# luntergroup/smcsmc

Hardware: AMD Instinct MI355X
Metric: genome segments/sec per EM iteration (Np=10000, 2 diploids, 100 Mb) (higher is better)
Workload: dtype f64

## Files before the change

include/smcsmc_pf.h:

```cpp
#ifndef SMCSMC_PF_H
#define SMCSMC_PF_H
#include <stdint.h>

#ifdef __cplusplus
extern "C" {
#endif

typedef struct pf_model {
    int32_t n_epochs;
    int32_t n_pops;
    int32_t nsam;
    int32_t flags;
    double loci_length;
    double mutation_rate;
    double recombination_rate;
    const double* change_times;
    const double* pop_sizes;
    const double* mig_rates;
    const double* single_mig;
    const int32_t* sample_pops;
    const int32_t* record_flags;
    const double* lags;
    int32_t n_bias_heights;
    int32_t delay_type;
// ... 8 lines not shown
    const double* rate_values;
    const double* leaf_rel_rates;
} pf_model;

typedef struct pf_params {
    int64_t np;
    double ess_fraction;
    uint64_t seed;
    int32_t max_trace_events;
    int32_t flags;
    int64_t log_cap;
    int64_t gen_cap;
    int64_t piece_cap;
    int32_t debug;
    int32_t mig_cap;
    int32_t count_wgs;
    int32_t delay_cap;
    int32_t count_workers;
    int32_t reserved4;
} pf_params;
#define PF_DEBUG_FORCE_LDS 1
#define PF_DEBUG_NO_FUSE   2
#define PF_DEBUG_NO_COUNT  4
#define PF_DEBUG_TWO_LAUNCH 8
#define PF_DEBUG_NO_SPEC_STAGE 32
#define PF_DEBUG_K_PIPE   16

#define PF_DEBUG_NO_DRAW_TABLE 128

#define PF_DEBUG_NO_SEARCH_LUT 256

#define PF_DEBUG_ONE_LAUNCH (1 << 23)

#define PF_DEBUG_NO_PAIR 4096
#define PF_DEBUG_FORCE_WIDE 2048

typedef struct pf_segments {
    int64_t n;
    const double* start;
    const double* length;
    const int8_t* state;
    const int8_t* alleles;
    const int32_t* max_record_epoch;
} pf_segments;

typedef struct pf_lookahead {
    int32_t level;
    int32_t max_doubletons;
    int32_t n_quantiles;
    int32_t flags;
    int64_t n;
    const double* first_singleton_distance;
    const double* relative_mutation_rate;
    const int8_t* is_singleton_unphased;
    const int32_t* n_doubletons;
    const int8_t* doubleton_idx;
    const double* doubleton_dist;
    const double* first_split_distance;
    const int8_t* split_alleles;
    const int32_t* split_count;
    const double* quantiles;
    const double* tbl_lengths;
    double mean_total_branch_length;
} pf_lookahead;
#define PF_LA_ROW_PIPELINE 1
#define PF_LA_ROW_PIPELINE_MP 2
// ... 92 lines not shown
```

profiles/gaps.py:

```python
#!/usr/bin/env python3
import csv
import glob
import statistics
import sys
from collections import defaultdict

path = glob.glob(sys.argv[1] + "/**/*kernel_trace.csv", recursive=True)[0]
rows = list(csv.DictReader(open(path)))
byq = defaultdict(list)
for r in rows:
    byq[r["Queue_Id"]].append((int(r["Start_Timestamp"]), int(r["End_Timestamp"]), r["Kernel_Name"].split("(")[0][:40]))
for q, ks in sorted(byq.items(), key=lambda kv: -len(kv[1]))[:3]:
    ks.sort()
    gaps = defaultdict(list)
    for (s0, e0, n0), (s1, e1, n1) in zip(ks, ks[1:]):
        gaps[(n0, n1)].append(s1 - e0)
    busy = sum(e - s for s, e, _ in ks)
    span = ks[-1][1] - ks[0][0]
    print("queue %s: %d kernels, busy %.1f ms of %.1f ms" % (q, len(ks), busy / 1e6, span / 1e6))
    for (a, b), g in sorted(gaps.items(), key=lambda kv: -len(kv[1]))[:6]:
        print("   %-40s -> %-40s n=%6d  gap mean %8.2f us  median %8.2f us" % (a, b, len(g), statistics.mean(g) / 1e3, statistics.median(g) / 1e3))
```

smcsmc_amd/csrc/pf_hip.hip:

```cpp
#include <hip/hip_runtime.h>
#include <type_traits>
#include <hip/hip_ext.h>

#include <algorithm>
#include <atomic>
#include <cmath>
#include <cstdio>
#include <cstdlib>
#include <cstring>
#include <mutex>
#include <string>
#include <vector>

#include "../../include/smcsmc_pf.h"
#include "pf_device.h"
#include "pf_types.h"
#include "pf_lane.h"
#include "pf_tree_reg.h"
#include "pf_look_reg.h"
#include "pf_lds_body.h"
#include "pf_mp_host.h"
#include "pf_wide_host.h"
#include "pf_pipe.h"
#include "pf_lds_pipe.h"
// ... 1370 lines not shown
#define PF_CNT_WIDE 128
#define PF_CNT_BATCH 2

template <int NI, int P, class KA>
__device__ __forceinline__ void count_run(AccT<P>& acc, const KA& A, const CountSrc& Q, const Win& W, const LMap& L, int g, long long i,
                                          int nr, const int* rst, const int* ran, double inv) {
    const long long Np = A.Np;
    int q0 = rst[i];
    int q1 = i + 1 < nr ? rst[i + 1] : (int)Np;
    long long a = ran[i];
    if (q1 <= q0 || q1 > (int)Np || q0 < 0 || a < 0 || a >= Np) return;
    const double* offp = Q.offp;
    const double* scp_ = Q.scanp;
    double hi = offp[(q1 - 1) >> 6] + scp_[q1 - 1];
    double lo = q0 > 0 ? offp[(q0 - 1) >> 6] + scp_[q0 - 1] : 0.0;
    double w = (hi - lo) * inv;
    if (!(w > 0.0)) return;
    unsigned k0 = A.gstart[(size_t)(g % A.Gcap) * Np + a];
    unsigned k1 = A.gstart[(size_t)((g + 1) % A.Gcap) * Np + a];
    if (Q.widx_live[a] - k0 > A.cap || k1 - k0 > A.cap) { if (!A.ctrl->err) A.ctrl->err = ERR_LOG_OVERFLOW; return; }
    records_contrib<NI, P>(acc, A, W, L, w, a, k0, k1);
}

struct FlatTask { double w; int a; unsigned k0; };
__device__ __forceinline__ FlatTask* count_flat_tasks() {
    __shared__ FlatTask ft[PF_BS];
    return ft;
}
__device__ __forceinline__ int* count_flat_prefix() {
    __shared__ int pre[PF_BS + 1];
    return pre;
}

template <int NM, int P, bool EXACT = false, class KA>
__device__ __forceinline__ void count_body(const KA& A, const CountSrc& Q, int e, double win_a, double win_b, int bx, int nbxg) {
    constexpr int NI = NM - 1;
    using AC = AccT<P>;
    constexpr int LDS_BYTES = (int)(((sizeof(AC) * (PF_BS / 64) + 15) & ~(size_t)15) + sizeof(int) * (PF_CNT_TILE + 1 + PF_BS / 64) + 16);
    char* const cl = count_lds<LDS_BYTES>();
    AC* const red = (AC*)cl;
    int* const s_off = (int*)(cl + ((sizeof(AC) * (PF_BS / 64) + 15) & ~(size_t)15));
    int* const s_wsum = s_off + PF_CNT_TILE + 1;
    const long long Np = A.Np;
    const int n = EXACT ? NM : A.n;
    const int G = Q.G;
    const double inv = Q.inv;
    Win W;
    W.e = e; W.rf = A.recflags[e];
    W.T0 = A.T[e]; W.T1 = e + 1 < A.E ? A.T[e + 1] : PF_INF;
    W.a_e = win_a; W.b_e = win_b;
    W.end_seq = (A.L == W.b_e);
    double* const s_lbins = count_bins();
    LMap L;
    L.lds = s_lbins; L.b0 = (long long)(W.a_e / 100.0); L.gopp = A.lmap_opp; L.gcnt = A.lmap_cnt; L.nbins = A.lmap_bins;
    {
        const long long span = (long long)(W.b_e / 100.0) - L.b0 + 4;
        L.nlds = span < 1 ? 1 : (span > PF_LBINS ? PF_LBINS : (int)span);
        L.ncnt = (A.n + 3) * L.nlds <= PF_LBINS ? L.nlds : 0;
    }
    bool bins_ready = false;
    const int g_lo = Q.g_lo, g_hi = Q.g_hi;
    if (g_hi < g_lo) return;
    const int lane = threadIdx.x & 63;
    const long long gtid = (long long)bx * PF_BS + threadIdx.x;
    const long long nthreads = (long long)nbxg * PF_BS;
    AC acc;
#pragma unroll
    for (int k = 0; k < AC::NC; ++k) acc.v[k] = 0.0;
    for (int tile_hi = g_hi; tile_hi >= g_lo; tile_hi -= PF_CNT_TILE) {
        const int tile_lo = tile_hi - PF_CNT_TILE + 1 > g_lo ? tile_hi - PF_CNT_TILE + 1 : g_lo;
// ... 116 lines not shown
                const double* rec = rec_ptr(A, a_r, s_ft[lo_j].k0 + (unsigned)(r - s_fpre[lo_j]));
                double f0 = rec[0], f1 = rec[1], f2 = rec[2], f3 = rec[3], f4 = rec[4];
                double S[NI];
#pragma unroll
                for (int q = 0; q < NI; ++q) S[q] = q < n - 1 ? rec[5 + q] : 0.0;
                unsigned long long dw = 0;
                if constexpr (NI >= PF_NMAX) if (L.gopp) dw = (unsigned long long)__double_as_longlong(rec[4 + n]);
                record_contrib_one<NI, P>(acc, A, W, L, w_r, a_r, f0, f1, f2, f3, f4, S, dw);
            }
            __syncthreads();
        }
    }
    if (L.gopp && bins_ready) {
        __syncthreads();
        for (int k = threadIdx.x; k < L.nlds; k += PF_BS) {
            double v = s_lbins[k];
            long long idx = L.b0 + k;
            if (v != 0.0 && idx < L.nbins) atomicAdd(&L.gopp[idx], v);
        }
        for (int k = threadIdx.x; k < (A.n + 2) * L.ncnt; k += PF_BS) {
            const double v = s_lbins[L.nlds + k];
            const long long idx = L.b0 + k % L.ncnt;
            if (v != 0.0 && idx < L.nbins) atomicAdd(&L.gcnt[(size_t)(k / L.ncnt) * L.nbins + idx], v);
        }
    }
#pragma unroll
    for (int k = 0; k < AC::NC; ++k) acc.v[k] = wave_tree_sum(acc.v[k]);
    if ((threadIdx.x & 63) == 0) red[threadIdx.x >> 6] = acc;
    __syncthreads();
    if (threadIdx.x < AC::NC) {
        const int k = threadIdx.x;
        double t = red[0].v[k];
        for (int w = 1; w < PF_BS / 64; ++w) t += red[w].v[k];
        A.partial[((size_t)e * A.nbx + bx) * AC::NC + k] += t;
    }
}


template <int NM, int P>
__global__ __launch_bounds__(PF_BS) void k_count(KArgs A, int e0, Windows Wn) {
    const int e = e0 + (int)blockIdx.y;
    if (e < Wn.first || e >= A.E) return;
    count_body<NM, P>(A, count_src_parity(A, A.sp, e), e, Wn.a[e], Wn.b[e], (int)blockIdx.x, (int)gridDim.x);
}

template <int NM, int P>
__global__ __launch_bounds__(PF_BS) void k_count_cw(KArgs A, int e0, Windows Wn) {
    const int e = e0 + (int)blockIdx.y;
    if (e < Wn.first || e >= A.E) return;
    const int j = A.E - 1 - e;
    const int cnb = A.cw_off[j + 1] - A.cw_off[j];
    if ((int)blockIdx.x >= cnb) return;
    count_body<NM, P>(A, count_src_parity(A, A.sp, e), e, Wn.a[e], Wn.b[e], (int)blockIdx.x, cnb);
}

template <int NM, bool BIASED, bool EXACT, bool TREES = false>
__global__ __launch_bounds__(PF_BS) void k_row(KArgs A, long long s, int fuse, int nb, int count_first, Windows Wprev) {
    if ((int)blockIdx.x < nb) {
        extend_reg_body<NM, BIASED, EXACT, TREES>(A, s, fuse);
    } else {
        const int idx = (int)blockIdx.x - nb;
        const int e = count_first + idx / nb;
        if (e < Wprev.first || e >= A.E) return;
        count_body<NM, 1, EXACT>(A, count_src_parity(A, A.sp ^ 1, e), e, Wprev.a[e], Wprev.b[e], idx % nb, nb);
    }
}

// ... 248 lines not shown
        c->gen_prev = c->gen; c->nres_prev = c->n_resample;
        if (PL.b_set_cur >= 0) c->cur = PL.b_set_cur;
    }
}

template <class KA>
__device__ __forceinline__ void draw_role(const KA& A, int tb, int nT, int par) {
    const long long Np = A.Np;
    const unsigned long long* c_in = A.dt_ctr + (size_t)(par ^ 1) * Np;
    const unsigned long long* f_in = A.dt_filled + (size_t)(par ^ 1) * Np;
    unsigned long long* f_out = A.dt_filled + (size_t)par * Np;
    const unsigned long long seed = A.seed;
    for (long long p = (long long)tb * PF_BS + threadIdx.x; p < Np; p += (long long)nT * PF_BS) {
        const unsigned long long c0 = c_in[p], f_old = f_in[p];
        const unsigned long long to = c0 + PF_DRAW_RING;
        double2* tab = (double2*)A.dt_tab + (size_t)p * PF_DRAW_RING;
        for (unsigned long long cc = f_old > c0 ? f_old : c0; cc < to; ++cc) {
            double u0, u1;
            philox_pair(seed, (unsigned)p, 0u, cc, u0, u1);
            tab[(unsigned)cc & (PF_DRAW_RING - 1)] = make_double2(u0, -dlog(u1));
        }
        f_out[p] = to;
    }
}

template <class KA>
__device__ __forceinline__ void pipe_ledger_item(const KA& A, const PipeLaunch& PL, const Ctrl::RowInfo& r, int lb) {
    const RunLists src = run_lists(A, r.lver), dst = run_lists(A, r.lver ^ 1);
    const int nblk = PL.nblk;
    if (lb < nblk) ledger_new_list(A, dst, A.rg_blkcnt + (size_t)PL.lc_slot * nblk * A.blk_gran, nblk, lb, r.gen, A.blk_gran);
    else ledger_update(A, lb - nblk, PL.nL - nblk, r.gen, r.g_retain, src, dst);
}

template <int NM, bool EXACT, int P, class KA>
__device__ __forceinline__ void pipe_count_item(const KA& A, const PipeLaunch& PL, const Ctrl::RowInfo& r, int idx) {
    int e, cbx, cnb;
    if (A.cw_off && !(A.flags & 512)) {
        int j = 0, hi = A.E;
        while (hi - j > 1) { const int mid = (j + hi) >> 1; if (A.cw_off[mid] <= idx) j = mid; else hi = mid; }
        e = A.E - 1 - j; cbx = idx - A.cw_off[j]; cnb = A.cw_off[j + 1] - A.cw_off[j];
    } else {
        e = (A.flags & 512) ? r.first + idx / PL.ncw : A.E - 1 - idx / PL.ncw;
        cbx = idx % PL.ncw; cnb = PL.ncw;
    }
    if (e >= A.E || e < r.first) return;
    if (A.flags & (1 << 22)) return;
    const DState st = state_slot(A, PL.lc_slot);
    CountSrc Q;
    Q.w = st.w_post; Q.S = st.S; Q.xm = st.x_mark; Q.ml = st.mark_limit;
    Q.widx = A.rg_widx + (size_t)PL.lc_slot * A.Np;
    Q.widx_live = A.rg_widx + (size_t)PL.live_slot * A.Np;
    Q.scanp = A.rg_scanp + (size_t)PL.lc_slot * A.Np;
    Q.offp = A.rg_coffp + (size_t)PL.lc_slot * A.nc;
    Q.lists = run_lists(A, r.lver);
    Q.inv = r.inv_T; Q.G = r.gen; Q.g_lo = r.g_lo[e]; Q.g_hi = r.g_hi[e];
    count_body<NM, P, EXACT>(A, Q, e, r.wa[e], r.wb[e], cbx, cnb);
}

template <int NM, bool BIASED, bool EXACT, bool TREES, int P = 1, bool BLC = false, bool QUEUE = false, bool LEAN = false, bool NO_EXTEND = false, bool LOOK = false, class KA>
__device__ __forceinline__ void pipe_roles(const KA& A, long long s, const PipeLaunch& PL, const Windows& Wb) {
    const int bx = pf_bx();
    const int nb = PL.nb;
    if constexpr (!LEAN) {
        if (bx < nb) {
            if constexpr (P == 1 && !BLC && !NO_EXTEND) { if (PL.row.extend || PL.row.complete) extend_reg_body<NM, BIASED, EXACT, TREES, true, false, LOOK>(A, s, 0, PL.row); }
            return;
        }
        if (bx == nb) {
            if (PL.b_slot < 0) return;
            extern __shared__ double smem[];
            PipeLds q = pipe_carve(smem + (2 * PF_EPAD + A.E + 2 * PF_BIAS_MAX + 3), A.nc);
            pipe_bookkeeping<BIASED>(A, q, PL, Wb);
            return;
        }
        if (bx - (nb + 1) < PL.nT) {
            if constexpr (P == 1 && !BLC) draw_role(A, bx - (nb + 1), PL.nT, PL.row.draws - 1);
            return;
        }
    } else {
        if (bx <= nb) return;
    }
    if (PL.lc_slot < 0 || PL.nL < -1) return;
    const Ctrl* c = A.ctrl;
    const Ctrl::RowInfo& r = c->ri[PL.lc_slot];
    const int lb = bx - (nb + 1) - PL.nT;
    if constexpr (!QUEUE) {
        if (lb < PL.nL) { if (r.flag) pipe_ledger_item(A, PL, r, lb); }
        else pipe_count_item<NM, EXACT, P>(A, PL, r, lb - PL.nL);
    } else {
        __shared__ int s_wk[8];
        if (lb >= PL.workers) return;
        if (threadIdx.x == 0) { s_wk[0] = PL.lc_slot; s_wk[1] = PL.live_slot; s_wk[2] = PL.nL; s_wk[3] = PL.nblk; s_wk[4] = PL.ncw; }
        const KA* Ap = &A;
        for (;;) {
            asm volatile("" : "+s"(Ap));
            const KA& A2 = *Ap;
            __syncthreads();
            if (threadIdx.x == 0) s_wk[6] = (int)__hip_atomic_fetch_add(&A2.ctrl->wq[s_wk[0]], 1u, __ATOMIC_RELAXED, __HIP_MEMORY_SCOPE_AGENT);
            __syncthreads();
            PipeLaunch Q2;
            Q2.lc_slot = s_wk[0]; Q2.live_slot = s_wk[1]; Q2.nL = s_wk[2]; Q2.nblk = s_wk[3]; Q2.ncw = s_wk[4];
            const int it = s_wk[6];
            const Ctrl::RowInfo& r2 = A2.ctrl->ri[Q2.lc_slot];
            const int ncnt = r2.first < A2.E ? (A2.cw_off ? A2.cw_off[A2.E - r2.first] : (A2.E - r2.first) * Q2.ncw) : 0;
            if (it >= ncnt + (r2.flag ? Q2.nL : 0)) return;
            if (it < ncnt) pipe_count_item<NM, EXACT, P>(A2, Q2, r2, it);
            else pipe_ledger_item(A2, Q2, r2, it - ncnt);
        }
    }
}

template <int NM, bool BIASED, bool EXACT, bool TREES>
__global__ __launch_bounds__(PF_BS) void k_pipe(KArgs A, long long s, PipeLaunch PL, Windows Wb) {
    pipe_roles<NM, BIASED, EXACT, TREES>(A, s, PL, Wb);
}

template <class KA>
__device__ __forceinline__ void sweep_windows(const KA& A, Ctrl* c, double pos, Windows& W) {
    const int e = threadIdx.x, E = A.E;
    if (e < 64) {
        const bool in = e < E;
// ... 57 lines not shown
        PipeLaunch PL;
        if (sweep_plan(ch, s, nb, PL)) {
            if (ch.split == 2) PL.nL = -3;
            if (pf_bx() == nb && PL.b_slot >= 0) sweep_windows(A, A.ctrl, PL.b_pos, W);
            pipe_roles<NM, BIASED, EXACT, TREES, 1, false, QUEUE, false, HEAD, LOOK>(A, s, PL, W);
        }
    }
    if constexpr (TRACE) {
        __syncthreads();
        if (threadIdx.x == 0) if (unsigned long long* w = wg_trace_slot(ch, t)) w[1] = wall_clock64();
    }
}
template <int NM, bool BIASED, bool EXACT, bool TREES, bool LOOK = false>
__global__ __launch_bounds__(PF_BS) void k_sweep(const SweepChunk* tab_g, long long t, int nb) {
    sweep_kernel_body<NM, BIASED, EXACT, TREES, false, false, false, LOOK>(tab_g, t, nb);
}
template <bool EXACT, bool TREES>
__global__ __launch_bounds__(PF_BS) __attribute__((amdgpu_waves_per_eu(3, 3))) void k_sweep4(const SweepChunk* tab_g, long long t, int nb) {
    sweep_kernel_body<4, false, EXACT, TREES, false, false, true>(tab_g, t, nb);
}
template <bool EXACT>
__global__ __launch_bounds__(PF_BS) void k_sweep4p(const SweepChunk* tab_g, long long t, int nb) {
    sweep_kernel_body<4, false, EXACT, false, false, false, true, false, true>(tab_g, t, nb);
}
template <bool EXACT, bool TRACE>
__global__ __launch_bounds__(PF_BS) __attribute__((amdgpu_waves_per_eu(3, 3))) void k_sweep4q(const SweepChunk* tab_g, long long t, int nb) {
    sweep_kernel_body<4, false, EXACT, false, TRACE, true, true>(tab_g, t, nb);
}
template <bool EXACT>
__global__ __launch_bounds__(PF_BS) __attribute__((amdgpu_waves_per_eu(3, 3))) void k_sweep4t(const SweepChunk* tab_g, long long t, int nb) {
    sweep_kernel_body<4, false, EXACT, false, true, false, true>(tab_g, t, nb);
}

template <int NM, int P, bool BIASED, bool EXACT = false, bool LEAN = false, bool QUEUE = false>
__device__ __forceinline__ void sweep_blc_body(const SweepChunk* tab_g, long long t) {
    SweepChunkC* tab = (SweepChunkC*)tab_g;
    SweepChunkC& ch = tab[pf_chunk()];
    KArgsC& A = ch.A;
    const long long s = ch.s_begin + t;
    __shared__ Windows W;
    Ctrl* c = A.ctrl;
    PipeLaunch PL;
    if (sweep_plan(ch, s, 0, PL)) {
        PL.nT = 0;
        if (ch.split == 2) PL.b_slot = -1;
        if (pf_bx() == 0 && PL.b_slot >= 0) sweep_windows(A, c, PL.b_pos, W);
        pipe_roles<NM, BIASED, EXACT, false, P, true, QUEUE, LEAN>(A, s, PL, W);
    }
}

template <int NM, int P, bool BIASED>
__global__ __launch_bounds__(PF_BS) void k_sweep_blc(const SweepChunk* tab_g, long long t) {
    sweep_blc_body<NM, P, BIASED>(tab_g, t);
}
template <bool EXACT>
__global__ __launch_bounds__(PF_BS) __attribute__((amdgpu_waves_per_eu(4, 4))) void k_sweep_blc4(const SweepChunk* tab_g, long long t) {
    sweep_blc_body<4, 1, false, EXACT, true>(tab_g, t);
}
template <bool EXACT>
__global__ __launch_bounds__(PF_BS) __attribute__((amdgpu_waves_per_eu(4, 4))) void k_sweep_blc4q(const SweepChunk* tab_g, long long t) {
    sweep_blc_body<4, 1, false, EXACT, true, true>(tab_g, t);
}

template <bool BIASED>
__global__ __launch_bounds__(PF_BS) void k_sweep_xl(const SweepChunk* tab_g, long long t) {
    SweepChunkC* tab = (SweepChunkC*)tab_g;
    SweepChunkC& ch = tab[pf_chunk()];
    KArgsC& A = ch.A;
    const long long s = ch.s_begin + t;
    PipeLaunch PL;
    if (!sweep_plan(ch, s, 0, PL)) return;
    if (!(PL.row.extend || PL.row.complete)) return;
    extern __shared__ double smem[];
    extend_lds_pipe_body<BIASED>(A, s, PL.row, smem);
}

__global__ void k_sweep_seed(const SweepChunk* tab_g) {
    SweepChunkC* tab = (SweepChunkC*)tab_g;
    SweepChunkC& ch = tab[blockIdx.x];
    KArgsC& A = ch.A;
    if (ch.s_last < ch.s_begin) return;
    Ctrl* c = A.ctrl;
    const int slot = (int)((ch.s_begin + PF_RING - 1) & (PF_RING - 1));
    if (threadIdx.x == 0) {
        Ctrl::RowInfo& r = c->ri[slot];
        r.n_res = c->n_resample; r.gen = c->gen; r.flag = 0; r.lver = c->lver; r.g_retain = c->g_retain; r.first = A.E;
        r.inv_T = 1.0; r.T = 1.0; r.S1 = 0.0; r.u = 0.0; r.pos = c->cur_pos;
        c->xr[slot].n_res = c->n_resample; c->xr[slot].gen = c->gen; c->xr[slot].flag = 0;
    }
    if ((int)threadIdx.x < A.E) c->counted_to[threadIdx.x] = ch.counted_to[threadIdx.x];
// ... 383 lines not shown
```

smcsmc_amd/csrc/pf_pipe.h:

```cpp
#pragma once
#include <cstddef>
#include <cstring>
#include <type_traits>

#include "pf_device.h"
#include "pf_types.h"

#define PF_PIPE_BS 256

__device__ __forceinline__ KArgsC& pf_reopen(KArgsC& A) { KArgsC* q = &A; asm volatile("" : "+s"(q)); return *q; }
__device__ __forceinline__ const KArgs& pf_reopen(const KArgs& A) { return A; }

#define PF_PIPE_STAGE 16
struct RowDecision { double T, S1, S2, ess, inv, u; int flag; };
struct PipeLds {
    double* l2s;
    double* pmx;
    double* l2_post; double* l2_sq; double* l2_tot;
    double* wredd;
    double* stage;
    int* slo;
    int* wint;
};
__host__ __device__ inline size_t pipe_lds_doubles(int nc) {
// ... 194 lines not shown
        else if constexpr (L == 1) return (unsigned)l1[K];
        else if constexpr (L == 2) return (unsigned)l2[K];
        else if constexpr (L == 3) return (unsigned)l3[K];
        else return (unsigned)l4[K];
    }
    template <int OFF> __device__ __forceinline__ unsigned long long dword() const {
        return ((unsigned long long)word<OFF + 4>() << 32) | (unsigned long long)word<OFF>();
    }
};
#define PF_HP(R, f) ((__attribute__((address_space(1))) std::remove_pointer_t<decltype(SweepHead::f)>*)(R).template dword<(int)offsetof(SweepHead, f)>())
#define PF_HL(R, f) ((long long)(R).template dword<(int)offsetof(SweepHead, f)>())
#define PF_HI(R, f) ((int)(R).template word<(int)offsetof(SweepHead, f)>())

inline SweepHead sweep_head_entry(const KArgs& A, const SweepChunk& ch, int phase) {
    SweepHead H;
    memset(&H, 0, sizeof(H));
    const size_t sp = (size_t)((ch.s_begin + phase + PF_RING - 1) & (PF_RING - 1)), Np = (size_t)A.Np, nc = (size_t)A.nc;
    H.s_begin = ch.s_begin; H.s_last = ch.s_last; H.Np = A.Np;
    H.nc = A.nc; H.n = A.n; H.E = A.E; H.flags = A.flags; H.nT = ch.nT; H.split = ch.split; H.nblk = ch.nblk; H.no_count = ch.no_count; H.P = A.P;
    H.slot_prev = (int)sp;
    H.cpost = A.rg_cpost + sp * nc; H.csq = A.rg_csq + sp * nc; H.cpil = A.rg_cpil + sp * nc; H.cmx1 = A.rg_cmx1 + sp * nc;
    H.last1 = &A.ctrl->last1[sp]; H.xr_before = &A.ctrl->xr[(sp + PF_RING - 1) & (PF_RING - 1)];
    H.scan1m = A.rg_scan1m + sp * Np; H.rg_widx = A.rg_widx + sp * Np;
    const DState st = state_slot(A, (int)sp);
    H.S = st.S; H.C = st.C; H.w_post = st.w_post; H.w_pilot = st.w_pilot; H.next_base = st.next_base; H.x_mark = st.x_mark;
    H.mark_limit = st.mark_limit; H.Ltree = st.Ltree;
    H.widx = A.widx; H.rng_ctr = A.rng_ctr; H.ebuf = A.ebuf;
    H.dt_filled = A.dt_filled ? A.dt_filled + (size_t)((ch.s_begin + phase + 1) & 1) * Np : nullptr;
    H.seg_start = A.seg_start; H.seg_len = A.seg_len; H.seg_limit = A.seg_limit; H.seg_state = A.seg_state; H.seg_alleles = A.seg_alleles;
    H.T = A.T; H.Hc = A.Hc; H.inv2N = A.inv2N; H.lut = A.lut; H.ctrl = A.ctrl;
    return H;
}

template <class KA>
__device__ __forceinline__ double sweep_seg_pos(const KA& A, long long s) {
    const double e = A.seg_start[s] + A.seg_len[s];
    return e < A.L ? e : A.L;
}

__device__ __forceinline__ bool sweep_plan(SweepChunkC& ch, long long s, int nb, PipeLaunch& PL) {
    const long long s_begin = ch.s_begin, s_last = ch.s_last;
    if (s_last < s_begin || s > s_last + 2) return false;
    const bool extend = s <= s_last, flush1 = s == s_last + 1;
    const bool have_b = extend ? (s > s_begin) : flush1;
    const bool have_lc = extend ? (s > s_begin + 1) : (flush1 ? (s_last - 1 >= s_begin) : true);
    PL.nb = nb; PL.nblk = ch.nblk;
    PL.row.extend = extend ? 1 : 0;
    PL.row.complete = ((extend && s > s_begin) || flush1) ? 1 : 0;
    PL.row.slot_prev = PL.row.complete ? (int)((s - 1) & (PF_RING - 1)) : -1;
    PL.row.slot_out = (int)(s & (PF_RING - 1));
    PL.row.pos_prev = (PL.row.complete && s > s_begin) ? sweep_seg_pos(ch.A, s - 1) : 0.0;
    PL.row.draws = ch.nT > 0 ? 1 + (int)(s & 1) : 0;
    PL.ahead = PL.row.ahead = (ch.split || ch.A.P > 1) ? 1 : 0;
    PL.nT = extend ? ch.nT : 0;
    PL.b_slot = have_b ? (int)((s - 1) & (PF_RING - 1)) : -1;
    PL.b_row = s - 1;
    PL.b_pos = have_b ? sweep_seg_pos(ch.A, s - 1) : 0.0;
    PL.b_set_cur = flush1 ? (int)((s_last + 1) & (PF_RING - 1)) : -1;
    PL.lc_slot = (have_lc && !ch.no_count) ? (int)((s - 2) & (PF_RING - 1)) : -1;
    PL.live_slot = (int)((s - 1) & (PF_RING - 1));
    PL.nL = PL.lc_slot >= 0 ? ch.nL_full : 0;
    PL.ncw = ch.ncw;
    PL.workers = ch.workers;
    return true;
}
```

smcsmc_amd/csrc/pf_run.h:

```cpp

static Windows host_windows(pf_handle* h, double current_base, bool end_data) {
    const int E = h->E;
    Windows W;
    memset(&W, 0, sizeof(W));
    W.first = E;
    W.end_data = end_data ? 1 : 0;
    for (int e = 0; e < E; ++e) {
        double lagging = end_data ? 0.0 : h->h_lags[e];
        double x_end = current_base - lagging;
        W.a[e] = h->h_counted_to[e];
        if ((x_end - h->h_counted_to[e]) < lagging * 0.1 && W.first > e) {
            W.b[e] = h->h_counted_to[e];
        } else {
            W.b[e] = x_end;
            W.first = std::min(W.first, e);
        }
    }
    for (int e = 0; e < E; ++e) h->h_counted_to[e] = W.b[e];
    return W;
}

static bool timing_on(pf_handle* h, long long s) { return h->timing_period > 0 && (s % h->timing_period) == 0; }

static Windows no_windows(pf_handle* h) {
// ... 391 lines not shown
            ch.s_last = last;
            for (int q = 0; q < h->E; ++q) ch.counted_to[q] = g->h_counted_to[q];
            ch.no_count = g->no_count ? 1 : 0;
            ch.nL_full = nL_full;
            ch.ncw = g->ncw;
            ch.nblk = g->nblocks;
            ch.nT = (g->A.dt_tab && g->P == 1) ? g->nblocks : 0;
            ch.split = split;
            ch.workers = g->workers;
            ch.trace = h->d_trace; ch.trace_t0 = h->trace_t0; ch.trace_n = h->d_trace ? h->trace_n : 0; ch.trace_stride = h->trace_stride;
            if (last >= s_begin) steps = std::max(steps, last - s_begin + 3);
        }
        if (steps == 0) return 0;
        const size_t head_bytes = sizeof(SweepHead) * PF_RING * (size_t)nh, chunk_bytes = sizeof(SweepChunk) * (size_t)nh;
        h->h_table.assign(head_bytes + chunk_bytes, 0);
        SweepHead* heads_end = (SweepHead*)(h->h_table.data() + head_bytes);
        if (h->P == 1 && h->n <= 4 && !is_biased(h))
            for (int k = 0; k < nh; ++k)
                for (int j = 0; j < PF_RING; ++j) *sweep_head_of(heads_end, k, j) = sweep_head_entry(h->h_sweep[k].A, h->h_sweep[k], j);
        memcpy(h->h_table.data() + head_bytes, h->h_sweep.data(), chunk_bytes);
        if (hipMemcpyAsync((char*)h->d_sweep - head_bytes, h->h_table.data(), head_bytes + chunk_bytes, hipMemcpyHostToDevice, h->stream) != hipSuccess) {
            g_err = "upload of the chunk table failed"; return -1;
        }
        hipLaunchKernelGGL(k_sweep_seed, dim3(nh), dim3(PF_BS), 0, h->stream, h->d_sweep);
        if (two_streams) {
            seeded = next_sync_event(h);
            hipEventRecord(seeded, h->stream);
        }
        W1.resize((size_t)nh); W2.resize((size_t)nh);
        for (int k = 0; k < nh; ++k) { W1[k] = no_windows(hs[k]); W2[k] = W1[k]; }
        return 1;
    }
    void ring_wait(long long t) const {
        static_assert(PF_RING == 16, "the wait schedule is written for sixteen ring slots");
        if (t >= 8 && (t & 7) == 0) hipStreamWaitEvent(h->stream, h->ev_blc[(size_t)((t - 7) & 15)], 0);
    }
    hipEvent_t x_done(long long t) const { return h->ev_x[(size_t)(t & 15)]; }
    hipEvent_t blc_done(long long t) const { return h->ev_blc[(size_t)(t & 15)]; }
    int lc_wgs(long long t) const {
        int columns = 0;
        bool any_lc = false;
        for (int k = 0; k < nh; ++k)
            if (t >= 2 && s_begin + t - 2 <= h->h_sweep[k].s_last && !hs[k]->no_count) { any_lc = true; columns = std::max(columns, h->E - W2[k].first); }
        const int workers = h->h_sweep[0].workers;
        return workers > 0 ? (any_lc ? workers : 0) : nL_full + h->cw_off[columns];
    }
    void step_done(long long t) {
        if ((t & 1023) == 1023) trim_spans(h);
        const long long s = s_begin + t;
        for (int k = 0; k < nh; ++k) {
            pf_handle* g = hs[k];
            W2[k] = W1[k];
            if (s <= h->h_sweep[k].s_last) {
                W1[k] = host_windows(g, seg_pos(g, s), false);
                g->step_windows = W1[k];
                if (W1[k].first < g->E && !g->no_count) g->fin_pending = true;
            } else {
                W1[k] = no_windows(g);
            }
        }
    }
    int leave() {
        h->k_launches[0] -= 2;
        if (two_streams) hipStreamWaitEvent(h->stream, blc_done(steps - 1), 0);
        for (int k = 0; k < nh; ++k) {
            pf_handle* g = hs[k];
            const long long last = h->h_sweep[k].s_last;
            if (last >= s_begin) g->seg_done = last + 1;
            if (k > 0) {
// ... 26 lines not shown
            Timed tm(h, 0, timing_on(h, s_begin + t));
            launch_sweep(h, grid, t);
        }
        if (check_launch("k_sweep")) return -1;
        F.step_done(t);
    }
    return F.leave();
}

static int run_sweep_split(pf_handle* const* hs, int nh, long long s_begin, long long s_end) {
    if (s_begin >= s_end) return 0;
    SweepFrame F(hs, nh, s_begin, true);
    pf_handle* h = F.h;
    const int nb = F.nb;
    if (F.join()) return -1;
    if (const int rc = F.table(s_end, 2); rc <= 0) return rc;
    const int nbp = (int)((h->Np + PF_PAIR_N - 1) / PF_PAIR_N);
    bool paired = !dbg(h, PF_DEBUG_NO_PAIR) && (long long)nh * nbp <= pf_device_cus(h->device);
    for (int k = 0; k < nh; ++k) if (hs[k]->A.vb_coal || dbg(hs[k], PF_DEBUG_NO_PAIR)) paired = false;
    for (int k = 0; k < nh; ++k) hs[k]->row_form = paired ? PF_ROW_FORM_PAIRED : PF_ROW_FORM_SINGLE;
    const int nbx = paired ? nbp : nb;
    if (paired && !h->pair_lds_set) {
        hipError_t rc = hipSuccess;
        with_row_instance(h, [&](auto NM, auto BIASED, auto EXACT, auto TREES) {
            if constexpr (NM == 4 && !BIASED && !TREES) rc = hipFuncSetAttribute((const void*)k_sweep4p<EXACT>, hipFuncAttributeMaxDynamicSharedMemorySize, (int)h->smem_pipe);
        });
        if (rc != hipSuccess) { g_err = "k_sweep4p: the LDS of the paired row kernel was refused (PF_DEBUG_NO_PAIR runs the other form)"; return -1; }
        h->pair_lds_set = true;
    }
    const dim3 gx((unsigned)(nbx + 1 + h->h_sweep[0].nT), (unsigned)nh), blk(PF_BS);
    const long long batch = std::max(1, std::min(4, h->split_batch > 0 ? h->split_batch : 4));
    std::vector<unsigned> pending_grid((size_t)batch, 1u);
    const bool queue = h->h_sweep[0].workers > 0;
    hipStreamWaitEvent(h->cstream, F.seeded, 0);
    for (long long t = 0; t < F.steps; ++t) {
        F.ring_wait(t);
        const bool batch_end = ((t + 1) % batch) == 0 || t == F.steps - 1;
        {
            Timed tm(h, 0, timing_on(h, s_begin + t));
            with_row_instance(h, [&](auto NM, auto BIASED, auto EXACT, auto TREES) {
                if constexpr (NM == 4 && !BIASED && !TREES) {
                    if (paired) {
                        if (batch_end) hipExtLaunchKernelGGL((k_sweep4p<EXACT>), gx, blk, h->smem_pipe, h->stream, nullptr, F.x_done(t), 0, h->d_sweep, t, nbx);
                        else hipLaunchKernelGGL((k_sweep4p<EXACT>), gx, blk, h->smem_pipe, h->stream, h->d_sweep, t, nbx);
                    } else if (batch_end) hipExtLaunchKernelGGL((k_sweep4<EXACT, false>), gx, blk, h->smem_pipe, h->stream, nullptr, F.x_done(t), 0, h->d_sweep, t, nb);
                    else hipLaunchKernelGGL((k_sweep4<EXACT, false>), gx, blk, h->smem_pipe, h->stream, h->d_sweep, t, nb);
                }
            });
        }
        if (check_launch(paired ? "k_sweep4p (extend, bookkeeping and draw roles)" : "k_sweep4 (extend, bookkeeping and draw roles)")) return -1;
        pending_grid[(size_t)(t % batch)] = (unsigned)(1 + F.lc_wgs(t));
        if (batch_end) {
            hipStreamWaitEvent(h->cstream, F.x_done(t), 0);
            for (long long u = t - (t % batch); u <= t; ++u) {
                const dim3 grid(pending_grid[(size_t)(u % batch)], (unsigned)nh);
                with_row_instance(h, [&](auto NM, auto BIASED, auto EXACT, auto TREES) {
                    if constexpr (NM == 4 && !BIASED && !TREES) {
                        if (queue) hipExtLaunchKernelGGL((k_sweep_blc4q<EXACT>), grid, blk, 0, h->cstream, nullptr, F.blc_done(u), 0, h->d_sweep, u);
                        else hipExtLaunchKernelGGL((k_sweep_blc4<EXACT>), grid, blk, 0, h->cstream, nullptr, F.blc_done(u), 0, h->d_sweep, u);
                    }
                });
            }
            if (check_launch("k_sweep_blc (ledger and count roles)")) return -1;
        }
        F.step_done(t);
    }
    return F.leave();
}

static int run_sweep_x(pf_handle* const* hs, int nh, long long s_begin, long long s_end, RunPath path) {
    if (s_begin >= s_end) return 0;
    const bool xl = path == RunPath::SweepXl;
    SweepFrame F(hs, nh, s_begin, true);
    pf_handle* h = F.h;
    if (F.join()) return -1;
    if (const int rc = F.table(s_end, xl ? 1 : 0); rc <= 0) return rc;
    for (long long t = 0; t < F.steps; ++t) {
        F.ring_wait(t);
        {
            Timed tm(h, 0, timing_on(h, s_begin + t));
            if (xl) {
                const dim3 gx((unsigned)F.nb, (unsigned)nh), bx(PF_BS);
                if (is_biased(h)) hipExtLaunchKernelGGL((k_sweep_xl<true>), gx, bx, h->smem_sweep_x, h->stream, nullptr, F.x_done(t), 0, h->d_sweep, t);
                else hipExtLaunchKernelGGL((k_sweep_xl<false>), gx, bx, h->smem_sweep_x, h->stream, nullptr, F.x_done(t), 0, h->d_sweep, t);
            } else {
                pf_mp_launch_sweep_x(h->A, h->d_sweep, nh, t, h->smem_sweep_x, h->stream, F.x_done(t));
            }
        }
        if (check_launch(xl ? "k_sweep_xl" : "k_sweep_xmp")) return -1;
        hipStreamWaitEvent(h->cstream, t >= 1 ? F.x_done(t - 1) : F.seeded, 0);
        const dim3 grid((unsigned)(1 + F.lc_wgs(t)), (unsigned)nh), blk(PF_BS);
        with_blc_instance(h, [&](auto NM, auto P, auto BIASED) {
// ... 83 lines not shown
```

smcsmc_amd/pf.py:

```python
import ctypes as C
import os

import numpy as np

_HERE = os.path.dirname(os.path.abspath(__file__))
LIB_PATH = os.path.join(_HERE, "csrc", "libsmcsmc_pf.so")
_LIB = None


class PfError(RuntimeError):
    pass


class _Model(C.Structure):
    _fields_ = [
        ("n_epochs", C.c_int32), ("n_pops", C.c_int32), ("nsam", C.c_int32), ("flags", C.c_int32),
        ("loci_length", C.c_double), ("mutation_rate", C.c_double), ("recombination_rate", C.c_double),
        ("change_times", C.POINTER(C.c_double)), ("pop_sizes", C.POINTER(C.c_double)),
        ("mig_rates", C.POINTER(C.c_double)), ("single_mig", C.POINTER(C.c_double)),
        ("sample_pops", C.POINTER(C.c_int32)), ("record_flags", C.POINTER(C.c_int32)),
        ("lags", C.POINTER(C.c_double)),
        ("n_bias_heights", C.c_int32), ("delay_type", C.c_int32),
        ("bias_heights", C.POINTER(C.c_double)), ("bias_strengths", C.POINTER(C.c_double)),
        ("application_delays", C.POINTER(C.c_double)),
# ... 235 lines not shown
def probe_tree_edit(S, Cc, h, lin, rp, sb, tc, u_attach, device=0):
    L = load_library()
    f8 = lambda a, shape: np.ascontiguousarray(a, dtype=np.float64).reshape(shape)
    i4 = lambda a, shape: np.ascontiguousarray(a, dtype=np.int32).reshape(shape)
    n = len(h)
    a = [f8(S, (n, 3)), i4(Cc, (n, 6)), f8(h, n), i4(lin, n), i4(rp, n), i4(sb, n), f8(tc, n), f8(u_attach, n)]
    oi = np.zeros((2, n, 10), np.int32); od = np.zeros((2, n, 4), np.float64)
    rc = L.pf_probe_tree_edit(n, *[x.ctypes.data for x in a], oi.ctypes.data, od.ctypes.data, int(device))
    if rc != 0:
        raise PfError("pf_probe_tree_edit failed (%d)" % rc)
    return oi, od


WAVE_PRIMS_D = ("wave_tree_sum", "wave_hs_scan", "wave_max_scan_d", "wave_prev_lane")
WAVE_PRIMS_I = ("wave_max_scan_i", "wave_minmax.min", "wave_minmax.max", "wave_prev_lane")


def probe_wave_prims(xd, xi, device=0):
    L = load_library()
    xd = np.ascontiguousarray(xd, dtype=np.float64); xi = np.ascontiguousarray(xi, dtype=np.int32)
    if xd.ndim != 2 or xd.shape[1] != 64 or xi.shape != xd.shape:
        raise PfError("probe_wave_prims: xd and xi must both be [K][64]")
    k = xd.shape[0]
    od = np.zeros((2, 4, k, 64), np.float64); oi = np.zeros((2, 4, k, 64), np.int32)
    rc = L.pf_probe_wave_prims(k, xd.ctypes.data, xi.ctypes.data, od.ctypes.data, oi.ctypes.data, int(device))
    if rc != 0:
        raise PfError("pf_probe_wave_prims failed (%d)" % rc)
    return od, oi


RUN_PATHS = ("General", "TwoLaunch", "KPipe", "Sweep", "SweepSplit", "SweepXmp", "SweepXl")
ROW_FORMS = (None, "single", "paired")
DEBUG_NO_PAIR = 4096


class ParticleFilter:
    def __init__(self, model, np_particles, ess_fraction=0.5, seed=1, max_trace_events=64, device=0, local_recomb=False,
                 record_trees=False, log_cap=0, gen_cap=0, piece_cap=0, debug=0, mig_cap=0, count_wgs=0, delay_cap=0,
                 delay_evict=False, count_workers=0):
        self.L = load_library()
        self._pack(model, np_particles, ess_fraction, seed, max_trace_events, local_recomb, record_trees, log_cap, gen_cap, piece_cap, debug,
                   mig_cap, count_wgs, delay_cap, delay_evict, count_workers)
        self.h = self.L.pf_create(C.byref(self._model), C.byref(self._params), int(device))
        if not self.h:
            raise PfError(_err(self.L))
        self.n_segs = 0

    def _pack(self, model, np_particles, ess_fraction=0.5, seed=1, max_trace_events=64, local_recomb=False, record_trees=False, log_cap=0,
              gen_cap=0, piece_cap=0, debug=0, mig_cap=0, count_wgs=0, delay_cap=0, delay_evict=False, count_workers=0):
        m = model
        self._ct = np.ascontiguousarray(m["change_times"], dtype=np.float64)
        E = len(self._ct)
        P = int(m.get("n_pops", 1))
        self._ps = np.ascontiguousarray(m["pop_sizes"], dtype=np.float64).reshape(E * P)
        self._rf = np.ascontiguousarray(m.get("record_flags", [3] * E), dtype=np.int32)
        self._lags = np.ascontiguousarray(m["lags"], dtype=np.float64)
        flags = (1 if m.get("ancestral_aware") else 0) | (2 if m.get("dephase") else 0)
        self.E, self.P, self.nsam, self.Np = E, P, int(m["nsam"]), int(np_particles)
        self.max_trace_events = int(max_trace_events)
        self._model = _Model(E, P, self.nsam, flags, float(m["loci_length"]), float(m["mutation_rate"]),
                             float(m["recombination_rate"]), _dp(self._ct), _dp(self._ps), None, None, None,
                             self._rf.ctypes.data_as(C.POINTER(C.c_int32)), _dp(self._lags))
        _attach_bias(self, self._model, m)
        _attach_structure(self, self._model, m, E, P)
        self.loci_length = float(m["loci_length"])
        self._params = _Params(self.Np, float(ess_fraction), int(seed), self.max_trace_events,
# ... 320 lines not shown
```

Baseline: 47200.

## Record completion events only for awaited count launches and slim the count kernel

In the split sweep path, the count-role launches now attach a completion event only when a later ring wait actually depends on that step (or when a debug flag forces it). All other count launches use a plain launch without an event. The count kernel gets a counts-only specialisation: it skips the row-end position loads and the windows setup, and it reads the partial accumulator at entry so the end does a plain store instead of a read-modify-write. The aim is to cut per-launch event overhead and the serial scalar loads at kernel entry, at the cost of a hard-coded wait schedule that both host and device must keep in step.

```diff
diff --git a/include/smcsmc_pf.h b/include/smcsmc_pf.h
--- a/include/smcsmc_pf.h
+++ b/include/smcsmc_pf.h
@@ -64,6 +64,7 @@
 
 #define PF_DEBUG_ONE_LAUNCH (1 << 23)
 
+#define PF_DEBUG_SIGNAL_ALL_COUNTS 16384
 #define PF_DEBUG_NO_PAIR 4096
 #define PF_DEBUG_FORCE_WIDE 2048
 
diff --git a/profiles/count_chain_isa.py b/profiles/count_chain_isa.py
--- /dev/null
+++ b/profiles/count_chain_isa.py
@@ -0,0 +1,80 @@
+#!/usr/bin/env python3
+import os
+import re
+import subprocess
+import sys
+import tempfile
+
+sys.path.insert(0, os.path.join(os.path.dirname(os.path.abspath(__file__)), "..", "tests", "tools"))
+sys.path.insert(0, os.path.join(os.path.dirname(os.path.abspath(__file__)), ".."))
+from smcsmc_amd import build
+
+KERNELS = {"k_sweep_blc4<true>": "_Z12k_sweep_blc4ILb1EEvPK10SweepChunkx", "k_sweep_blc4<false>": "_Z12k_sweep_blc4ILb0EEvPK10SweepChunkx"}
+TARGET = "hipv4-amdgcn-amd-amdhsa--gfx950"
+
+
+def tool(name):
+    hipcc = os.path.realpath(build._hipcc())
+    root = os.path.dirname(os.path.dirname(hipcc))
+    for d in (os.path.dirname(hipcc), os.path.join(root, "lib", "llvm", "bin"), os.path.join(root, "llvm", "bin")):
+        if os.path.exists(os.path.join(d, name)):
+            return os.path.join(d, name)
+    raise SystemExit(name + " not found beside hipcc")
+
+
+def code_object(obj, tmp, tag):
+    fat, co = os.path.join(tmp, tag + ".hipfb"), os.path.join(tmp, tag + ".co")
+    subprocess.check_call([tool("llvm-objcopy"), "--dump-section", ".hip_fatbin=" + fat, obj, os.path.join(tmp, tag + ".copy.o")])
+    subprocess.check_call([tool("clang-offload-bundler"), "--unbundle", "--type=o", "--input=" + fat, "--targets=" + TARGET, "--output=" + co])
+    return co
+
+
+def listing(co, sym):
+    text = subprocess.check_output([tool("llvm-objdump"), "-d", "--no-show-raw-insn", "--disassemble-symbols=" + sym, co], text=True)
+    return [re.sub(r"\s*//.*$", "", ln).strip() for ln in text.splitlines() if re.match(r"^\s+[a-z]", ln)]
+
+
+def is_vmem(ins):
+    return ins.startswith(("global_", "flat_", "buffer_", "scratch_"))
+
+
+def describe(ins):
+    head = []
+    for i in ins:
+        if is_vmem(i):
+            break
+        head.append(i)
+    return dict(head=head, n=len(ins),
+                head_sloads=sum(1 for i in head if i.startswith("s_load")), head_waits=sum(1 for i in head if i.startswith("s_waitcnt") and "lgkmcnt(0)" in i),
+                sloads=sum(1 for i in ins if i.startswith("s_load")), waits=sum(1 for i in ins if i.startswith("s_waitcnt") and "lgkmcnt(0)" in i),
+                vm_loads=sum(1 for i in ins if is_vmem(i) and "_load" in i), barriers=sum(1 for i in ins if i.startswith("s_barrier")))
+
+
+def main():
+    import kernel_meta
+    sides = {"parent": sys.argv[1], "new": sys.argv[2]}
+    with tempfile.TemporaryDirectory() as tmp:
+        cos = {k: code_object(v, tmp, k) for k, v in sides.items()}
+        for name, sym in KERNELS.items():
+            d = {k: describe(listing(co, sym)) for k, co in cos.items()}
+            m = {k: kernel_meta.kernels(obj)[sym] for k, obj in sides.items()}
+            print("## `%s`\n" % name)
+            print("| | parent | new |\n|---|---|---|")
+            rows = [("instructions", "n"), ("scalar loads before the first vector memory instruction", "head_sloads"),
+                    ("`s_waitcnt lgkmcnt(0)` before the first vector memory instruction", "head_waits"), ("scalar loads, whole kernel", "sloads"),
+                    ("`s_waitcnt lgkmcnt(0)`, whole kernel", "waits"), ("vector loads, whole kernel", "vm_loads"), ("`s_barrier`", "barriers")]
+            for what, key in rows:
+                print("| %s | %d | %d |" % (what, d["parent"][key], d["new"][key]))
+            for what, key in (("VGPRs", "vgpr"), ("AGPRs", "agpr"), ("SGPRs", "sgpr"), ("static LDS, bytes", "lds"), ("scratch, bytes", "scratch")):
+                print("| %s | %d | %d |" % (what, m["parent"][key], m["new"][key]))
+            for k in ("parent", "new"):
+                print("\nThe entry, %s (scalar loads and waits in layout order up to the first vector memory instruction):\n\n```" % k)
+                for i in d[k]["head"]:
+                    if i.startswith(("s_load", "s_waitcnt", "s_cbranch", "s_branch", "s_endpgm")):
+                        print(i)
+                print("```")
+            print()
+
+
+if __name__ == "__main__":
+    main()
diff --git a/profiles/gaps.py b/profiles/gaps.py
--- a/profiles/gaps.py
+++ b/profiles/gaps.py
@@ -5,7 +5,13 @@
 import sys
 from collections import defaultdict
 
-path = glob.glob(sys.argv[1] + "/**/*kernel_trace.csv", recursive=True)[0]
+args = sys.argv[1:]
+by_grid = None
+if "--by-grid" in args:
+    i = args.index("--by-grid")
+    by_grid = args[i + 1]
+    del args[i:i + 2]
+path = glob.glob(args[0] + "/**/*kernel_trace.csv", recursive=True)[0]
 rows = list(csv.DictReader(open(path)))
 byq = defaultdict(list)
 for r in rows:
@@ -20,3 +26,18 @@
     print("queue %s: %d kernels, busy %.1f ms of %.1f ms" % (q, len(ks), busy / 1e6, span / 1e6))
     for (a, b), g in sorted(gaps.items(), key=lambda kv: -len(kv[1]))[:6]:
         print("   %-40s -> %-40s n=%6d  gap mean %8.2f us  median %8.2f us" % (a, b, len(g), statistics.mean(g) / 1e3, statistics.median(g) / 1e3))
+
+if by_grid:
+    dur = defaultdict(list)
+    for r in rows:
+        name = r["Kernel_Name"].split("(")[0]
+        if by_grid not in name:
+            continue
+        wgs = int(r["Grid_Size_X"]) // max(1, int(r["Workgroup_Size_X"]))
+        dur[(name[:40], wgs, int(r["Grid_Size_Y"]))].append(int(r["End_Timestamp"]) - int(r["Start_Timestamp"]))
+    total = sum(sum(d) for d in dur.values())
+    n_all = sum(len(d) for d in dur.values())
+    print("%s by grid: %d launches, %.1f ms, mean %.2f us" % (by_grid, n_all, total / 1e6, total / 1e3 / max(1, n_all)))
+    for (name, wgs, gy), d in sorted(dur.items()):
+        print("   %-40s grid %5d x %d  n=%6d  mean %8.2f us  median %8.2f us  min %7.2f  max %8.2f  %5.1f %% of its time" %
+              (name, wgs, gy, len(d), statistics.mean(d) / 1e3, statistics.median(d) / 1e3, min(d) / 1e3, max(d) / 1e3, 100.0 * sum(d) / max(1, total)))
diff --git a/smcsmc_amd/csrc/pf_hip.hip b/smcsmc_amd/csrc/pf_hip.hip
--- a/smcsmc_amd/csrc/pf_hip.hip
+++ b/smcsmc_amd/csrc/pf_hip.hip
@@ -1426,10 +1426,12 @@
     return pre;
 }
 
-template <int NM, int P, bool EXACT = false, class KA>
+template <int NM, int P, bool EXACT = false, bool ACC_AT_ENTRY = false, class KA>
 __device__ __forceinline__ void count_body(const KA& A, const CountSrc& Q, int e, double win_a, double win_b, int bx, int nbxg) {
     constexpr int NI = NM - 1;
     using AC = AccT<P>;
+    double acc_before = 0.0;
+    if constexpr (ACC_AT_ENTRY) { if (threadIdx.x < AC::NC) acc_before = A.partial[((size_t)e * A.nbx + bx) * AC::NC + threadIdx.x]; }
     constexpr int LDS_BYTES = (int)(((sizeof(AC) * (PF_BS / 64) + 15) & ~(size_t)15) + sizeof(int) * (PF_CNT_TILE + 1 + PF_BS / 64) + 16);
     char* const cl = count_lds<LDS_BYTES>();
     AC* const red = (AC*)cl;
@@ -1612,7 +1614,8 @@
         const int k = threadIdx.x;
         double t = red[0].v[k];
         for (int w = 1; w < PF_BS / 64; ++w) t += red[w].v[k];
-        A.partial[((size_t)e * A.nbx + bx) * AC::NC + k] += t;
+        if constexpr (ACC_AT_ENTRY) A.partial[((size_t)e * A.nbx + bx) * AC::NC + k] = acc_before + t;
+        else A.partial[((size_t)e * A.nbx + bx) * AC::NC + k] += t;
     }
 }
 
@@ -1927,7 +1930,7 @@
     else ledger_update(A, lb - nblk, PL.nL - nblk, r.gen, r.g_retain, src, dst);
 }
 
-template <int NM, bool EXACT, int P, class KA>
+template <int NM, bool EXACT, int P, bool ACC_AT_ENTRY = false, class KA>
 __device__ __forceinline__ void pipe_count_item(const KA& A, const PipeLaunch& PL, const Ctrl::RowInfo& r, int idx) {
     int e, cbx, cnb;
     if (A.cw_off && !(A.flags & 512)) {
@@ -1949,10 +1952,11 @@
     Q.offp = A.rg_coffp + (size_t)PL.lc_slot * A.nc;
     Q.lists = run_lists(A, r.lver);
     Q.inv = r.inv_T; Q.G = r.gen; Q.g_lo = r.g_lo[e]; Q.g_hi = r.g_hi[e];
-    count_body<NM, P, EXACT>(A, Q, e, r.wa[e], r.wb[e], cbx, cnb);
-}
-
-template <int NM, bool BIASED, bool EXACT, bool TREES, int P = 1, bool BLC = false, bool QUEUE = false, bool LEAN = false, bool NO_EXTEND = false, bool LOOK = false, class KA>
+    count_body<NM, P, EXACT, ACC_AT_ENTRY>(A, Q, e, r.wa[e], r.wb[e], cbx, cnb);
+}
+
+template <int NM, bool BIASED, bool EXACT, bool TREES, int P = 1, bool BLC = false, bool QUEUE = false, bool LEAN = false, bool NO_EXTEND = false, bool LOOK = false,
+          bool ACC_AT_ENTRY = false, class KA>
 __device__ __forceinline__ void pipe_roles(const KA& A, long long s, const PipeLaunch& PL, const Windows& Wb) {
     const int bx = pf_bx();
     const int nb = PL.nb;
@@ -1981,7 +1985,7 @@
     const int lb = bx - (nb + 1) - PL.nT;
     if constexpr (!QUEUE) {
         if (lb < PL.nL) { if (r.flag) pipe_ledger_item(A, PL, r, lb); }
-        else pipe_count_item<NM, EXACT, P>(A, PL, r, lb - PL.nL);
+        else pipe_count_item<NM, EXACT, P, ACC_AT_ENTRY>(A, PL, r, lb - PL.nL);
     } else {
         __shared__ int s_wk[8];
         if (lb >= PL.workers) return;
@@ -2105,7 +2109,7 @@
     sweep_kernel_body<4, false, EXACT, false, true, false, true>(tab_g, t, nb);
 }
 
-template <int NM, int P, bool BIASED, bool EXACT = false, bool LEAN = false, bool QUEUE = false>
+template <int NM, int P, bool BIASED, bool EXACT = false, bool LEAN = false, bool QUEUE = false, bool COUNTS_ONLY = false>
 __device__ __forceinline__ void sweep_blc_body(const SweepChunk* tab_g, long long t) {
     SweepChunkC* tab = (SweepChunkC*)tab_g;
     SweepChunkC& ch = tab[pf_chunk()];
@@ -2114,7 +2118,13 @@
     __shared__ Windows W;
     Ctrl* c = A.ctrl;
     PipeLaunch PL;
-    if (sweep_plan(ch, s, 0, PL)) {
+    if constexpr (COUNTS_ONLY) {
+        static_assert(LEAN && !QUEUE, "the second launch of a split step in its static form");
+        if (sweep_plan<false>(ch, s, 0, PL)) {
+            PL.nT = 0; PL.b_slot = -1;
+            pipe_roles<NM, BIASED, EXACT, false, P, true, false, true, false, false, true>(A, s, PL, W);
+        }
+    } else if (sweep_plan(ch, s, 0, PL)) {
         PL.nT = 0;
         if (ch.split == 2) PL.b_slot = -1;
         if (pf_bx() == 0 && PL.b_slot >= 0) sweep_windows(A, c, PL.b_pos, W);
@@ -2128,7 +2138,7 @@
 }
 template <bool EXACT>
 __global__ __launch_bounds__(PF_BS) __attribute__((amdgpu_waves_per_eu(4, 4))) void k_sweep_blc4(const SweepChunk* tab_g, long long t) {
-    sweep_blc_body<4, 1, false, EXACT, true>(tab_g, t);
+    sweep_blc_body<4, 1, false, EXACT, true, false, true>(tab_g, t);
 }
 template <bool EXACT>
 __global__ __launch_bounds__(PF_BS) __attribute__((amdgpu_waves_per_eu(4, 4))) void k_sweep_blc4q(const SweepChunk* tab_g, long long t) {
diff --git a/smcsmc_amd/csrc/pf_pipe.h b/smcsmc_amd/csrc/pf_pipe.h
--- a/smcsmc_amd/csrc/pf_pipe.h
+++ b/smcsmc_amd/csrc/pf_pipe.h
@@ -250,12 +250,21 @@
     return H;
 }
 
+inline long long sweep_ring_awaited(long long t) {
+    static_assert(PF_RING == 16, "the wait schedule is written for sixteen ring slots");
+    return (t >= 8 && (t & 7) == 0) ? t - 7 : -1;
+}
+inline bool sweep_blc_awaited(long long u, long long steps) {
+    return (u + 7 < steps && sweep_ring_awaited(u + 7) == u) || u == steps - 1;
+}
+
 template <class KA>
 __device__ __forceinline__ double sweep_seg_pos(const KA& A, long long s) {
     const double e = A.seg_start[s] + A.seg_len[s];
     return e < A.L ? e : A.L;
 }
 
+template <bool ROW_END = true>
 __device__ __forceinline__ bool sweep_plan(SweepChunkC& ch, long long s, int nb, PipeLaunch& PL) {
     const long long s_begin = ch.s_begin, s_last = ch.s_last;
     if (s_last < s_begin || s > s_last + 2) return false;
@@ -267,13 +276,13 @@
     PL.row.complete = ((extend && s > s_begin) || flush1) ? 1 : 0;
     PL.row.slot_prev = PL.row.complete ? (int)((s - 1) & (PF_RING - 1)) : -1;
     PL.row.slot_out = (int)(s & (PF_RING - 1));
-    PL.row.pos_prev = (PL.row.complete && s > s_begin) ? sweep_seg_pos(ch.A, s - 1) : 0.0;
+    PL.row.pos_prev = (ROW_END && PL.row.complete && s > s_begin) ? sweep_seg_pos(ch.A, s - 1) : 0.0;
     PL.row.draws = ch.nT > 0 ? 1 + (int)(s & 1) : 0;
     PL.ahead = PL.row.ahead = (ch.split || ch.A.P > 1) ? 1 : 0;
     PL.nT = extend ? ch.nT : 0;
     PL.b_slot = have_b ? (int)((s - 1) & (PF_RING - 1)) : -1;
     PL.b_row = s - 1;
-    PL.b_pos = have_b ? sweep_seg_pos(ch.A, s - 1) : 0.0;
+    PL.b_pos = (ROW_END && have_b) ? sweep_seg_pos(ch.A, s - 1) : 0.0;
     PL.b_set_cur = flush1 ? (int)((s_last + 1) & (PF_RING - 1)) : -1;
     PL.lc_slot = (have_lc && !ch.no_count) ? (int)((s - 2) & (PF_RING - 1)) : -1;
     PL.live_slot = (int)((s - 1) & (PF_RING - 1));
diff --git a/smcsmc_amd/csrc/pf_run.h b/smcsmc_amd/csrc/pf_run.h
--- a/smcsmc_amd/csrc/pf_run.h
+++ b/smcsmc_amd/csrc/pf_run.h
@@ -447,9 +447,9 @@
         return 1;
     }
     void ring_wait(long long t) const {
-        static_assert(PF_RING == 16, "the wait schedule is written for sixteen ring slots");
-        if (t >= 8 && (t & 7) == 0) hipStreamWaitEvent(h->stream, h->ev_blc[(size_t)((t - 7) & 15)], 0);
-    }
+        if (const long long u = sweep_ring_awaited(t); u >= 0) hipStreamWaitEvent(h->stream, blc_done(u), 0);
+    }
+    bool blc_awaited(long long u) const { return sweep_blc_awaited(u, steps); }
     hipEvent_t x_done(long long t) const { return h->ev_x[(size_t)(t & 15)]; }
     hipEvent_t blc_done(long long t) const { return h->ev_blc[(size_t)(t & 15)]; }
     int lc_wgs(long long t) const {
@@ -542,6 +542,7 @@
     const long long batch = std::max(1, std::min(4, h->split_batch > 0 ? h->split_batch : 4));
     std::vector<unsigned> pending_grid((size_t)batch, 1u);
     const bool queue = h->h_sweep[0].workers > 0;
+    const bool signal_all = dbg(h, PF_DEBUG_SIGNAL_ALL_COUNTS);
     hipStreamWaitEvent(h->cstream, F.seeded, 0);
     for (long long t = 0; t < F.steps; ++t) {
         F.ring_wait(t);
@@ -564,10 +565,14 @@
             hipStreamWaitEvent(h->cstream, F.x_done(t), 0);
             for (long long u = t - (t % batch); u <= t; ++u) {
                 const dim3 grid(pending_grid[(size_t)(u % batch)], (unsigned)nh);
+                const bool signal = signal_all || F.blc_awaited(u);
                 with_row_instance(h, [&](auto NM, auto BIASED, auto EXACT, auto TREES) {
                     if constexpr (NM == 4 && !BIASED && !TREES) {
-                        if (queue) hipExtLaunchKernelGGL((k_sweep_blc4q<EXACT>), grid, blk, 0, h->cstream, nullptr, F.blc_done(u), 0, h->d_sweep, u);
-                        else hipExtLaunchKernelGGL((k_sweep_blc4<EXACT>), grid, blk, 0, h->cstream, nullptr, F.blc_done(u), 0, h->d_sweep, u);
+                        if (queue) {
+                            if (signal) hipExtLaunchKernelGGL((k_sweep_blc4q<EXACT>), grid, blk, 0, h->cstream, nullptr, F.blc_done(u), 0, h->d_sweep, u);
+                            else hipLaunchKernelGGL((k_sweep_blc4q<EXACT>), grid, blk, 0, h->cstream, h->d_sweep, u);
+                        } else if (signal) hipExtLaunchKernelGGL((k_sweep_blc4<EXACT>), grid, blk, 0, h->cstream, nullptr, F.blc_done(u), 0, h->d_sweep, u);
+                        else hipLaunchKernelGGL((k_sweep_blc4<EXACT>), grid, blk, 0, h->cstream, h->d_sweep, u);
                     }
                 });
             }
diff --git a/smcsmc_amd/pf.py b/smcsmc_amd/pf.py
--- a/smcsmc_amd/pf.py
+++ b/smcsmc_amd/pf.py
@@ -291,6 +291,7 @@
 RUN_PATHS = ("General", "TwoLaunch", "KPipe", "Sweep", "SweepSplit", "SweepXmp", "SweepXl")
 ROW_FORMS = (None, "single", "paired")
 DEBUG_NO_PAIR = 4096
+DEBUG_SIGNAL_ALL_COUNTS = 16384
 
 
 class ParticleFilter:
```

Result: faster. 48210 (median of 6 runs) (+2.1%).
